# albertogp71/qLDPCsim

Hardware: AMD Instinct MI355X
Metric: decoded shots/sec (MS 50-iter, LP118_0) at 1/2/4/8 GPU; achieved HBM GB/s (higher is better)
Workload: dtype f32+f64

## Files before the change

### qldpcsim_amd/csrc/ms_flood_qc.h

```cpp

template <typename F, int... I>
__device__ __forceinline__ void static_for_seq(F&& f, std::integer_sequence<int, I...>) {
  (f(std::integral_constant<int, I>{}), ...);
}
template <int N, typename F>
__device__ __forceinline__ void static_for(F&& f) {
  static_for_seq(f, std::make_integer_sequence<int, N>{});
}

template <int N>
__device__ __forceinline__ float row_ror_f32(float x) {
  if constexpr ((N & 15) == 0) {
    return x;
  } else {
    return __builtin_bit_cast(float, __builtin_amdgcn_update_dpp(0, __builtin_bit_cast(int, x), 0x120 + (N & 15),
                                                                 0xf, 0xf, true));
  }
}

__device__ __forceinline__ uint32_t row_bits(uint64_t b, int rowsh) {
  const uint32_t half = (rowsh & 32) ? (uint32_t)(b >> 32) : (uint32_t)b;
  return (half >> (rowsh & 16)) & 0xffffu;
}

struct RowQueue {
  long long cur, end, rows, batch;
  uint32_t* q;
  uint32_t tk, tlen, seen;
  __device__ __forceinline__ RowQueue(const DecodeArgs& a, long long rows_, int lane)
      : cur(0), end(0), rows(rows_), batch(a.batch), q(a.queue), tk(0), tlen(1), seen(0) {
    if (q) claim(lane);
  }
  __device__ __forceinline__ void claim(int lane) {
    const long long rem = batch - rows - (long long)seen;
    long long len = rem / (4 * rows);
    len = len < 1 ? 1 : (len > 64 ? 64 : len);
    tlen = (uint32_t)len;
    if (lane == 0) tk = atomicAdd(q, tlen);
  }
  __device__ __forceinline__ long long take(int lane) {
    if (cur == end) {
      const uint32_t t = __builtin_amdgcn_readfirstlane(tk);
      seen = t + tlen;
      cur = uniform64(rows + (long long)t);
      end = uniform64(cur + tlen);
    }
    const long long h = cur;
    cur = uniform64(cur + 1);
    if (cur == end) claim(lane);
    return h;
  }
};

template <typename T, int B>
__device__ __forceinline__ uint32_t qc_check(const DecodeArgs& a, double L, float (&S)[T::NB],
                                             float (&c2v)[T::MB][T::DC], uint32_t synb, int& fl) {
  constexpr int DC = T::DC;
  static_for<DC>([&](auto E) __attribute__((always_inline)) {
    float &sx = S[T::cvar[B][E]], &cx = c2v[B][E];
    asm volatile("" : "+v"(sx), "+v"(cx));
  });
  double v[DC];
  uint32_t hv[DC], hp[DC];
  static_for<DC>([&](auto E) __attribute__((always_inline)) {
    constexpr int e = E, c = T::cvar[B][e], s = T::cshift[B][e];
    const double post = L + (double)row_ror_f32<(16 - s) & 15>(S[c]);
    v[e] = post - (double)c2v[B][e];
    hv[e] = hi_word(v[e]);
    hp[e] = hi_word(post);
  });
  double min1, min2;
  min12_tree<DC>(v, min1, min2);
  const uint32_t ph = xor_tree<DC>(hp);
  const uint32_t sh = xor_tree<DC>(hv);
  double m1 = min1, m2 = min2;
  if (__builtin_expect(ballot((min1 == 0.0) | (min2 == __builtin_inf())) != 0, 0)) {
    m1 = __builtin_isinf(min1) ? 0.0 : min1;
    m2 = __builtin_isinf(min2) ? 0.0 : min2;
    if (m1 == 0.0) fl |= FLAG_MIN_ZERO;
  }
  const uint32_t npm = ((sh >> 31) ^ synb) << 31;
  const uint32_t c1n = opaque_always(__builtin_bit_cast(uint32_t, (float)(a.beta * m1)) ^ npm);
  const uint32_t c2n = opaque_always(__builtin_bit_cast(uint32_t, (float)(a.beta * m2)) ^ npm);
  static_for<DC>([&](auto E) __attribute__((always_inline)) {
    constexpr int e = E;
    const uint32_t c = (__builtin_fabs(v[e]) == min1) ? c2n : c1n;
    c2v[B][e] = __builtin_bit_cast(float, c ^ (hv[e] & 0x80000000u));
  });
  uint32_t unsat = (ph >> 31) ^ synb;
  static_for<DC>([&](auto E) __attribute__((always_inline)) {
    float& cx = c2v[B][E];
    asm volatile("" : "+v"(cx));
  });
  asm volatile("" : "+v"(unsat));
  return unsat;
}

template <int N>
__device__ __forceinline__ uint32_t row_ror_u32(uint32_t x) {
  if constexpr ((N & 15) == 0) {
    return x;
  } else {
    return (uint32_t)__builtin_amdgcn_update_dpp(0, (int)x, 0x120 + (N & 15), 0xf, 0xf, true);
  }
}

template <typename T, int B>
__device__ __forceinline__ uint32_t qc_parity(const uint32_t (&hw)[(T::NB + 31) / 32], uint32_t synb) {
  uint32_t ph = synb;
  static_for<T::DC>([&](auto E) __attribute__((always_inline)) {
    constexpr int e = E, c = T::cvar[B][e], s = T::cshift[B][e];
    ph ^= row_ror_u32<(16 - s) & 15>(hw[c >> 5]) >> (c & 31);
  });
  ph &= 1u;
  asm volatile("" : "+v"(ph));
  return ph;
}

template <typename T, int C>
__device__ __forceinline__ float qc_colsum(const float (&c2v)[T::MB][T::DC]) {
  float s = row_ror_f32<T::vshift[C][0]>(c2v[T::vchk[C][0]][T::vslot[C][0]]);
  static_for<T::vdeg[C] - 1>([&](auto I) __attribute__((always_inline)) {
    constexpr int t = I + 1;
    s = s + row_ror_f32<T::vshift[C][t]>(c2v[T::vchk[C][t]][T::vslot[C][t]]);
  });
  return s;
}

template <typename T>
__device__ __forceinline__ void flood_qc_body(const DecodeArgs& a) {
  constexpr int MB = T::MB, NB = T::NB, DC = T::DC;
  static_assert(qc::kLift == 16, "one DPP row per half-shot");
  const int lane = threadIdx.x & 63;
  const int k = lane & 15, q = lane >> 4, rowsh = lane & 48;
  const int waves = blockDim.x >> 6;
  const long long rows = 4ll * gridDim.x * waves;
  const long long batch = a.batch;
  constexpr int n = 16 * NB, m = 16 * MB;
  constexpr int wn = (n + 63) / 64;

  float c2v[MB][DC], S[NB];
  int it = 0, fl = 0;
  uint32_t synreg = 0;
  long long hs = 4ll * ((long long)blockIdx.x * waves + (threadIdx.x >> 6)) + q;
  RowQueue Q(a, rows, lane);
  bool live = false, fin = true;
  bool conv = false;
  int iters = 0;
  bool started = false;

  for (;;) {
    const uint64_t finb = ballot_b(fin);
    if (finb != 0) {
      if (started) {
        if (fin) {
          const DecodeArgs& f = kargs_fresh();
          int kl = k, rsh = rowsh;
          asm volatile("" : "+v"(kl), "+v"(rsh));
          if (f.eh_bits) {
            uint32_t lo = 0, hi = 0;
            static_for<wn>([&](auto W) __attribute__((always_inline)) {
              uint32_t r[4] = {0, 0, 0, 0};
              static_for<4>([&](auto I) __attribute__((always_inline)) {
                constexpr int c = 4 * W + I;
                if constexpr (c < NB) r[I] = row_bits(ballot_b(a.L + (double)S[c] < 0.0), rsh);
              });
              if (kl == W) lo = r[0] | (r[1] << 16), hi = r[2] | (r[3] << 16);
            });
            if (kl < wn) ((uint64_t*)f.ehat)[hs * wn + kl] = ((uint64_t)hi << 32) | lo;
          } else {
            uint8_t* eo = f.ehat + hs * (long long)n + kl;
            static_for<NB>([&](auto C) __attribute__((always_inline)) {
              eo[16 * C] = (uint8_t)(a.L + (double)S[C] < 0.0);
            });
          }
          if (f.post) {
            double* po = f.post + hs * (long long)n + kl;
            static_for<NB>([&](auto C) __attribute__((always_inline)) { po[16 * C] = a.L + (double)S[C]; });
          }
          const bool mz = row_bits(ballot_b((fl & FLAG_MIN_ZERO) != 0), rsh) != 0;
          if (kl == 0) {
            f.iters[hs] = iters;
            if (f.flags) f.flags[hs] = (int32_t)((mz ? FLAG_MIN_ZERO : 0) | (conv ? FLAG_CONVERGED : 0));
          }
        }
        if (Q.q) {
#pragma unroll
          for (int r = 0; r < 4; ++r) {
            if ((finb >> (16 * r)) & 1u) {
              const long long h = Q.take(lane);
              if (q == r) hs = h;
            }
          }
        } else if (fin) {
          hs += rows;
        }
      }
      started = true;
      if (fin) {
        live = hs < batch;
        it = 0, synreg = 0;
        if (live) {
          const DecodeArgs& f = kargs_fresh();
          int kl = k;
          asm volatile("" : "+v"(kl));
          if (f.syn_bits) {
            const uint32_t* row = (const uint32_t*)((const uint64_t*)f.syn + hs * f.wm);
            uint32_t w[(MB + 1) / 2];
#pragma unroll
            for (int i = 0; i < (MB + 1) / 2; ++i) w[i] = row[i];
#pragma unroll
            for (int b = 0; b < MB; ++b) synreg |= ((w[b >> 1] >> (16 * (b & 1) + kl)) & 1u) << b;
          } else {
            const uint8_t* row = f.syn + hs * (long long)m + kl;
            uint32_t w[MB];
#pragma unroll
            for (int b = 0; b < MB; ++b) w[b] = row[16 * b];
#pragma unroll
            for (int b = 0; b < MB; ++b) synreg |= (w[b] & 1u) << b;
          }
        }
        const double vf = (double)a.L32;
        const double av = __builtin_fabs(vf);
        const uint32_t cb = __builtin_bit_cast(uint32_t, (float)(a.beta * av));
        const uint32_t neg = (uint32_t)(vf < 0.0);
        fl = av == 0.0 ? FLAG_MIN_ZERO : 0;
        static_for<MB>([&](auto B) __attribute__((always_inline)) {
          const uint32_t negprod = ((neg * DC) ^ (synreg >> B)) & 1u;
          const float val = __builtin_bit_cast(float, cb | ((neg ^ negprod) << 31));
          static_for<DC>([&](auto E) __attribute__((always_inline)) { c2v[B][E] = val; });
        });
        fin = false;
      }
    }
    if (ballot_b(live) == 0) break;

    if (live) {
      static_for<NB>([&](auto C) __attribute__((always_inline)) {
        float& sc = S[C];
        sc = qc_colsum<T, C>(c2v);
        asm volatile("" : "+v"(sc));
      });
      it += 1;
      if (it == a.max_iter) {
        uint32_t hw[(NB + 31) / 32] = {};
        static_for<NB>([&](auto C) __attribute__((always_inline)) {
          hw[C / 32] |= (hi_word(a.L + (double)S[C]) >> 31) << (C % 32);
        });
        uint32_t un = 0;
        static_for<MB>([&](auto B) __attribute__((always_inline)) {
          un |= qc_parity<T, B>(hw, (synreg >> B) & 1u);
        });
        fin = true, iters = it;
        conv = row_bits(ballot_b(un != 0), rowsh) == 0;
      }
    }
    if (live && !fin) {
      uint32_t unsat = 0;
      static_for<MB>([&](auto B) __attribute__((always_inline)) {
        unsat |= qc_check<T, B>(a, a.L, S, c2v, (synreg >> B) & 1u, fl);
      });
      if (row_bits(ballot_b(unsat != 0), rowsh) == 0) fin = true, conv = true, iters = it;
    }
  }
}
```

Baseline: 15.54 million.

## Precompute f64 posteriors for selected QC columns to cut per-edge conversions

For up to QLDPC_QC_NP columns, chosen by a compile-time saving score, the column sum is stored as a precomputed f64 posterior (L + sum) instead of an f32 sum. Check-node edges then rotate the f64 value with two DPP moves rather than redoing the f32-to-f64 conversion and add on every edge. This trades extra VGPRs (two per stored column) and extra DPP ops for fewer conversions. It also re-derives lane indices and kernel args via opaque reloads to reduce live registers across the loop.

```diff
diff --git a/qldpcsim_amd/csrc/ms_flood_qc.h b/qldpcsim_amd/csrc/ms_flood_qc.h
--- a/qldpcsim_amd/csrc/ms_flood_qc.h
+++ b/qldpcsim_amd/csrc/ms_flood_qc.h
@@ -18,6 +18,47 @@
   }
 }
 
+template <int N>
+__device__ __forceinline__ double row_ror_f64(double x) {
+  if constexpr ((N & 15) == 0) {
+    return x;
+  } else {
+    const uint64_t u = __builtin_bit_cast(uint64_t, x);
+    const uint32_t lo = (uint32_t)__builtin_amdgcn_update_dpp(0, (int)(uint32_t)u, 0x120 + (N & 15), 0xf, 0xf, true);
+    const uint32_t hi =
+        (uint32_t)__builtin_amdgcn_update_dpp(0, (int)(uint32_t)(u >> 32), 0x120 + (N & 15), 0xf, 0xf, true);
+    return __builtin_bit_cast(double, ((uint64_t)hi << 32) | lo);
+  }
+}
+
+#ifndef QLDPC_QC_NP
+#define QLDPC_QC_NP 34
+#endif
+template <typename T>
+constexpr int qc_np() { return QLDPC_QC_NP < T::NB ? QLDPC_QC_NP : T::NB; }
+
+template <typename T>
+constexpr int qc_post64_saving(int c) {
+  int zero = 0;
+  for (int t = 0; t < T::vdeg[c]; ++t) zero += T::vshift[c][t] == 0;
+  return 8 * T::vdeg[c] - 2 * (T::vdeg[c] - zero) - 8;
+}
+template <typename T>
+constexpr bool qc_post64(int c) {
+  int rank = 0;
+  for (int d = 0; d < T::NB; ++d) {
+    const int sd = qc_post64_saving<T>(d), sc = qc_post64_saving<T>(c);
+    rank += sd > sc || (sd == sc && d < c);
+  }
+  return rank < qc_np<T>();
+}
+
+template <typename T, int C>
+__device__ __forceinline__ double qc_post(double L, const float (&S)[T::NB], const double (&P)[T::NB]) {
+  if constexpr (qc_post64<T>(C)) return P[C];
+  else return L + (double)S[C];
+}
+
 __device__ __forceinline__ uint32_t row_bits(uint64_t b, int rowsh) {
   const uint32_t half = (rowsh & 32) ? (uint32_t)(b >> 32) : (uint32_t)b;
   return (half >> (rowsh & 16)) & 0xffffu;
@@ -53,18 +94,26 @@
 };
 
 template <typename T, int B>
-__device__ __forceinline__ uint32_t qc_check(const DecodeArgs& a, double L, float (&S)[T::NB],
+__device__ __forceinline__ uint32_t qc_check(const DecodeArgs& a, double L, float (&S)[T::NB], double (&P)[T::NB],
                                              float (&c2v)[T::MB][T::DC], uint32_t synb, int& fl) {
   constexpr int DC = T::DC;
   static_for<DC>([&](auto E) __attribute__((always_inline)) {
-    float &sx = S[T::cvar[B][E]], &cx = c2v[B][E];
-    asm volatile("" : "+v"(sx), "+v"(cx));
+    float& cx = c2v[B][E];
+    if constexpr (qc_post64<T>(T::cvar[B][E])) {
+      double& px = P[T::cvar[B][E]];
+      asm volatile("" : "+v"(px), "+v"(cx));
+    } else {
+      float& sx = S[T::cvar[B][E]];
+      asm volatile("" : "+v"(sx), "+v"(cx));
+    }
   });
   double v[DC];
   uint32_t hv[DC], hp[DC];
   static_for<DC>([&](auto E) __attribute__((always_inline)) {
     constexpr int e = E, c = T::cvar[B][e], s = T::cshift[B][e];
-    const double post = L + (double)row_ror_f32<(16 - s) & 15>(S[c]);
+    double post;
+    if constexpr (qc_post64<T>(c)) post = row_ror_f64<(16 - s) & 15>(P[c]);
+    else post = L + (double)row_ror_f32<(16 - s) & 15>(S[c]);
     v[e] = post - (double)c2v[B][e];
     hv[e] = hi_word(v[e]);
     hp[e] = hi_word(post);
@@ -132,7 +181,7 @@
   constexpr int MB = T::MB, NB = T::NB, DC = T::DC;
   static_assert(qc::kLift == 16, "one DPP row per half-shot");
   const int lane = threadIdx.x & 63;
-  const int k = lane & 15, q = lane >> 4, rowsh = lane & 48;
+  const int q = lane >> 4, rowsh = lane & 48;
   const int waves = blockDim.x >> 6;
   const long long rows = 4ll * gridDim.x * waves;
   const long long batch = a.batch;
@@ -140,6 +189,7 @@
   constexpr int wn = (n + 63) / 64;
 
   float c2v[MB][DC], S[NB];
+  double P[NB];
   int it = 0, fl = 0;
   uint32_t synreg = 0;
   long long hs = 4ll * ((long long)blockIdx.x * waves + (threadIdx.x >> 6)) + q;
@@ -155,15 +205,16 @@
       if (started) {
         if (fin) {
           const DecodeArgs& f = kargs_fresh();
-          int kl = k, rsh = rowsh;
-          asm volatile("" : "+v"(kl), "+v"(rsh));
+          int ln = threadIdx.x;
+          asm volatile("" : "+v"(ln));
+          const int kl = ln & 15, rsh = ln & 48;
           if (f.eh_bits) {
             uint32_t lo = 0, hi = 0;
             static_for<wn>([&](auto W) __attribute__((always_inline)) {
               uint32_t r[4] = {0, 0, 0, 0};
               static_for<4>([&](auto I) __attribute__((always_inline)) {
                 constexpr int c = 4 * W + I;
-                if constexpr (c < NB) r[I] = row_bits(ballot_b(a.L + (double)S[c] < 0.0), rsh);
+                if constexpr (c < NB) r[I] = row_bits(ballot_b(qc_post<T, c>(a.L, S, P) < 0.0), rsh);
               });
               if (kl == W) lo = r[0] | (r[1] << 16), hi = r[2] | (r[3] << 16);
             });
@@ -171,12 +222,12 @@
           } else {
             uint8_t* eo = f.ehat + hs * (long long)n + kl;
             static_for<NB>([&](auto C) __attribute__((always_inline)) {
-              eo[16 * C] = (uint8_t)(a.L + (double)S[C] < 0.0);
+              eo[16 * C] = (uint8_t)(qc_post<T, C>(a.L, S, P) < 0.0);
             });
           }
           if (f.post) {
             double* po = f.post + hs * (long long)n + kl;
-            static_for<NB>([&](auto C) __attribute__((always_inline)) { po[16 * C] = a.L + (double)S[C]; });
+            static_for<NB>([&](auto C) __attribute__((always_inline)) { po[16 * C] = qc_post<T, C>(a.L, S, P); });
           }
           const bool mz = row_bits(ballot_b((fl & FLAG_MIN_ZERO) != 0), rsh) != 0;
           if (kl == 0) {
@@ -202,8 +253,9 @@
         it = 0, synreg = 0;
         if (live) {
           const DecodeArgs& f = kargs_fresh();
-          int kl = k;
-          asm volatile("" : "+v"(kl));
+          int ln = threadIdx.x;
+          asm volatile("" : "+v"(ln));
+          const int kl = ln & 15;
           if (f.syn_bits) {
             const uint32_t* row = (const uint32_t*)((const uint64_t*)f.syn + hs * f.wm);
             uint32_t w[(MB + 1) / 2];
@@ -220,9 +272,10 @@
             for (int b = 0; b < MB; ++b) synreg |= (w[b] & 1u) << b;
           }
         }
-        const double vf = (double)a.L32;
+        const DecodeArgs& g = kargs_fresh();
+        const double vf = (double)g.L32;
         const double av = __builtin_fabs(vf);
-        const uint32_t cb = __builtin_bit_cast(uint32_t, (float)(a.beta * av));
+        const uint32_t cb = __builtin_bit_cast(uint32_t, (float)(g.beta * av));
         const uint32_t neg = (uint32_t)(vf < 0.0);
         fl = av == 0.0 ? FLAG_MIN_ZERO : 0;
         static_for<MB>([&](auto B) __attribute__((always_inline)) {
@@ -237,15 +290,21 @@
 
     if (live) {
       static_for<NB>([&](auto C) __attribute__((always_inline)) {
-        float& sc = S[C];
-        sc = qc_colsum<T, C>(c2v);
-        asm volatile("" : "+v"(sc));
+        if constexpr (qc_post64<T>(C)) {
+          double& pc = P[C];
+          pc = a.L + (double)qc_colsum<T, C>(c2v);
+          asm volatile("" : "+v"(pc));
+        } else {
+          float& sc = S[C];
+          sc = qc_colsum<T, C>(c2v);
+          asm volatile("" : "+v"(sc));
+        }
       });
       it += 1;
       if (it == a.max_iter) {
         uint32_t hw[(NB + 31) / 32] = {};
         static_for<NB>([&](auto C) __attribute__((always_inline)) {
-          hw[C / 32] |= (hi_word(a.L + (double)S[C]) >> 31) << (C % 32);
+          hw[C / 32] |= (hi_word(qc_post<T, C>(a.L, S, P)) >> 31) << (C % 32);
         });
         uint32_t un = 0;
         static_for<MB>([&](auto B) __attribute__((always_inline)) {
@@ -258,7 +317,7 @@
     if (live && !fin) {
       uint32_t unsat = 0;
       static_for<MB>([&](auto B) __attribute__((always_inline)) {
-        unsat |= qc_check<T, B>(a, a.L, S, c2v, (synreg >> B) & 1u, fl);
+        unsat |= qc_check<T, B>(a, a.L, S, P, c2v, (synreg >> B) & 1u, fl);
       });
       if (row_bits(ballot_b(unsat != 0), rowsh) == 0) fin = true, conv = true, iters = it;
     }
```

Measured after the change: 16.93 million, median of 6. +8.9%, better.
